# vicchu/land_trendr

Hardware: AMD Instinct MI355X
Metric: Mpixels/sec full analyze (30-yr series) (higher is better)
Workload: dtype f64

## Files before the change

### land_trendr_amd/csrc/lt_fast.h

```cpp
#pragma once
#ifndef __HIPCC_RTC__
#include <type_traits>
#endif

#include "lt_pixel.h"

#ifndef LT_WB
#define LT_WB 8
#endif
#ifndef LT_RESOLVE_PRIV_MAXY
#define LT_RESOLVE_PRIV_MAXY 48
#endif
#ifndef LT_RESOLVE_FULL
#define LT_RESOLVE_FULL 1
#endif
#ifndef LT_AB_NO_YEAR_STORES
#define LT_AB_NO_YEAR_STORES 0
#endif
#ifndef LT_AB_NO_FITS
#define LT_AB_NO_FITS 0
#endif
#ifndef LT_AB_YEAR_SINK
#define LT_AB_YEAR_SINK 0
#endif
#ifndef LT_YEAR_NT
#define LT_YEAR_NT 1
#endif
#ifndef LT_YEAR_STORE_MODE
#define LT_YEAR_STORE_MODE 0
#endif

namespace lt {
__device__ inline void year_row_store(double v, double* a) {
#if LT_YEAR_STORE_MODE == 1
  asm volatile("global_store_dwordx2 %0, %1, off sc1" ::"v"(a), "v"(v) : "memory");
#elif LT_YEAR_STORE_MODE == 2
  asm volatile("global_store_dwordx2 %0, %1, off sc0 sc1" ::"v"(a), "v"(v) : "memory");
#elif LT_YEAR_STORE_MODE == 3
  asm volatile("global_store_dwordx2 %0, %1, off sc1 nt" ::"v"(a), "v"(v) : "memory");
#else
  __builtin_nontemporal_store(v, a);
#endif
}
}
#ifndef LT_CERT_RULES
#define LT_CERT_RULES 4
#endif
#ifndef LT_PASSB_SLOTS
#define LT_PASSB_SLOTS 3
#endif

#ifdef LT_SPEC_NRULES
#define LT_NRULES LT_SPEC_NRULES
#define LT_RULE(r) lt_spec_rules[r]
#define LT_PRE_MODE LT_SPEC_PRE_MODE
#else
#define LT_NRULES P.n_rules
#define LT_RULE(r) P.rules[r]
#define LT_PRE_MODE P.pre_threshold_mode
#endif
#ifdef LT_SPEC_LINE_COST
#define LT_LINE_COST LT_SPEC_LINE_COST
#else
#define LT_LINE_COST P.line_cost
#endif

namespace lt {

__device__ inline int dmul24(int m, int sxx, int sx) {
  return (int)(__umul24((unsigned)m, (unsigned)sxx) - __umul24((unsigned)sx, (unsigned)sx));
}

__device__ inline int wave_max(int v) {
#pragma unroll
  for (int o = 32; o > 0; o >>= 1) {
    const int u = __shfl_xor(v, o);
    v = u > v ? u : v;
  }
  return __builtin_amdgcn_readfirstlane(v);
}

template <class GX, class GY>
__device__ inline int lsq_lockstep(bool act, int m, GX X, GY Y, const lsq_xf* __restrict__ xtab,
                                   bool need_solution, bool need_ssr, double& slope, double& icpt,
                                   double& ssr) {
  const int key = act ? xset_key(m, X) : 0;
  const bool miss = act && key < 0;
  lsq_xf f;
  if (act && !miss) f = xtab[key];
  if (__ballot(miss)) {
    if (miss) lsq_factor(m, X, f);
  }
  slope = 0.0;
  icpt = 0.0;
  ssr = 0.0;
  return act ? lsq_apply(f, X, Y, need_solution, need_ssr, slope, icpt, ssr) : 0;
}

template <class GX, class GY>
__device__ inline int lsq_fit_lockstep(bool act, int m, GX X, GY Y,
                                       const lsq_xf* __restrict__ xtab, double& slope,
                                       double& icpt) {
  const int key = act ? xset_key(m, X) : 0;
  const bool miss = act && key < 0;
  lsq_xf f;
  if (act && !miss) f = xtab[key];
  if (__ballot(miss)) {
    if (miss) lsq_factor(m, X, f);
  }
  slope = 0.0;
  icpt = 0.0;
  int rc = 0;
  const bool big = act && m > 4;
  if (__ballot(big)) {
    if (big) {
      double ssr;
      rc = lsq_apply(f, X, Y, true, false, slope, icpt, ssr);
    }
  }
  if (act && m <= 4) rc = lsq_apply_small(f, X, Y, slope, icpt);
  return rc;
}

template <int MAXY, class VT, bool AGLDS>
struct WaveLds {
  VT ys[MAXY][64];
  uint8_t xn[MAXY][64];
  uint8_t ag[AGLDS ? MAXY : 1][64];
  int32_t year[LT_MAX_YEARS];
};

enum { kDone = 0, kDeferExact = 1, kDeferWide = 2 };

struct NoProbe {
  static constexpr int kStopAfter = -1;
  __device__ void mark(int) const {}
};

template <int MAXY, int RMAX, bool EXACT, class VT, class Probe = NoProbe>
__device__ inline int analyze_fast(const DevScene& S_launch, const lt_params& P, const lt_tile_in& in,
                                   const lt_tile_out& out, const lsq_xf* __restrict__ xtab,
                                   uint64_t* __restrict__ yflags, uint64_t* __restrict__ tl_bits,
                                   double* __restrict__ tl_eqn, int64_t p, bool live, int lane,
                                   WaveLds<MAXY, VT, EXACT>& L,
                                   const Probe& probe = Probe()) {
#ifdef LT_SPEC_SCENE
  const DevScene& S = lt_spec_scene;
  (void)S_launch;
#else
  const DevScene& S = S_launch;
#endif
#ifdef LT_SPEC_Y
  constexpr int Y = LT_SPEC_Y;
#else
  const int Y = S.n_years;
#endif
  const int64_t is = in.stride, os = out.stride;
  const double nan = __builtin_nan("");
  int status = LT_ST_OK;
  static_assert(LT_MAX_YEARS == 64, "one year-table word per lane");
  if (lane < Y) L.year[lane] = S.year[lane];
#ifdef LT_DEBUG_LDS_POISON
  for (int k = 0; k < MAXY; k++) {
    L.ys[k][lane] = (VT)(LT_DEBUG_LDS_POISON + 37 * k);
    L.xn[k][lane] = (uint8_t)(LT_DEBUG_LDS_POISON + 11 * k);
  }
#endif
  __syncthreads();

  int T = 0, y0 = 0;
  uint64_t pres = 0;
  constexpr bool kIntSeries = std::is_same<VT, int16_t>::value;
#if defined(LT_SPEC_YEAR_OUT) && LT_SPEC_YEAR_OUT == 0
  constexpr bool kFlatPick = true;
#else
  constexpr bool kFlatPick = false;
#endif
  double Ssum = 0.0, Qsum = 0.0;
  bool f32_bad = false;
  bool intdata = true;
  bool infdata = false;
  constexpr int WB = LT_WB;
#ifdef LT_SPEC_MASKED
  constexpr bool masked = LT_SPEC_MASKED != 0;
#ifdef LT_SPEC_VBITS
  constexpr bool vbits = masked && LT_SPEC_VBITS != 0;
#else
  const bool vbits = masked && in.obs_valid_bits != nullptr && S.n_obs <= 128;
#endif
#else
  const bool masked = in.obs_valid != nullptr || in.obs_valid_bits != nullptr;
  const bool vbits = in.obs_valid_bits != nullptr && S.n_obs <= 128;
#endif
  uint32_t vw0 = 0, vw1 = 0, vw2 = 0, vw3 = 0;
  if (vbits) {
    const uint32_t* vb = in.obs_valid_bits;
    const int64_t pq = live ? p : 0;
    const int nw = (S.n_obs + 31) >> 5;
    vw0 = vb[pq];
    if (nw > 1) vw1 = vb[is + pq];
    if (nw > 2) vw2 = vb[2 * is + pq];
    if (nw > 3) vw3 = vb[3 * is + pq];
  }
  for (int yb = 0; yb < Y; yb += WB) {
    int best[WB];
#pragma unroll
    for (int u = 0; u < WB; u++) {
      const int y = yb + u;
      best[u] = -1;
      if (y >= Y) continue;
      if (!masked) {
        best[u] = live ? S.winner_all[y] : -1;
        continue;
      }
      int bd = 0x7fffffff;
      const int k1 = S.slot_begin[y + 1];
      for (int k = S.slot_begin[y]; k < k1; k++) {
// ... 423 lines not shown
            const double den = md * D;
            double r = __builtin_amdgcn_rcp(den);
            r = __builtin_fma(r, __builtin_fma(-den, r, 1.0), r);
            e = __builtin_fma(t1, D, -(N1 * N1)) * r;
            e = e < 0.0 ? 0.0 : e;
          }
          const double v = (e + c) + oi;
          if (m >= 3) w = __builtin_fma(0x1p-50, __builtin_fabs(v), kScreen * Syy);
          if (v - w <= H) cand |= 1ull << i;
          H = v + w < H ? v + w : H;
          if (prune && m >= 3 && !__ballot(col && !(dp_start_bound(e, oi, 0.0, c, SyyAll) > H)))
            break;
        }
        const int nc = col ? __builtin_popcountll(cand) : 0;
        const int ncmax = wave_max(nc);
        double best = inf;
        int bi = 0;
        for (int r = 0; r < ncmax; r++) {
          const bool act = r < nc;
          const int i = act ? __builtin_ctzll(cand) : 0;
          if (act) cand &= cand - 1;
          const double oi = OPT[i];
          const int m = j - i + 1;
          const bool ls = act && m >= 3;
          double e = 0.0;
          if (__ballot(ls)) {
            double sm, sb, ssr;
            const int rc = lsq_lockstep(
                ls, m, [&](int k) { return (int)L.xn[i + k][lane]; },
                [&](int k) { return (double)L.ys[i + k][lane]; }, xtab, false, true, sm, sb, ssr);
            if (ls) {
              if (rc < 0) status |= LT_ST_NUMERIC;
              e = ssr;
            }
          }
          const double v = (e + c) + oi;
          if (act && v < best) {
            best = v;
            bi = i;
          }
        }
        if (col) {
          ag_set(j, bi);
          OPT[j + 1] = best;
        }
      }
    } else {
      const double c = LT_LINE_COST;
      const double inf = __builtin_inf();
      double OPT[MAXY + 1];
#pragma unroll
      for (int k = 0; k <= MAXY; k++) OPT[k] = 0.0;
      double SyyAll = 0.0;
      const bool prune = c >= 0.0;
      for (int jj = 0; jj < nmax; jj++) {
        const int j = __builtin_amdgcn_readfirstlane(jj);
        const bool col = j < n;
        double Sy = 0.0, Sxy = 0.0, Syy = 0.0;
        int Sx = 0, Sxx = 0;
        double H = inf;
        uint64_t cand = 0;
        {
          const double yj = (double)L.ys[j][lane];
          SyyAll = __builtin_fma(yj, yj, SyyAll);
        }
#pragma unroll
        for (int i = MAXY - 1; i >= 0; i--) {
          if (i > j) continue;
          const int xi = L.xn[i][lane];
          const double yi = (double)L.ys[i][lane];
          Sx += xi;
          Sxx += xi * xi;
          Sy += yi;
          Sxy = __builtin_fma((double)xi, yi, Sxy);
          Syy = __builtin_fma(yi, yi, Syy);
          const int m = j - i + 1;
          double e = 0.0, w = 0.0;
          if (m >= 3) {
            const double md = (double)m;
            const double D = (double)(m * Sxx - Sx * Sx);
            const double t1 = __builtin_fma(md, Syy, -(Sy * Sy));
            const double N1 = __builtin_fma(md, Sxy, -((double)Sx * Sy));
            const double den = md * D;
            double r = __builtin_amdgcn_rcp(den);
            r = __builtin_fma(r, __builtin_fma(-den, r, 1.0), r);
            e = __builtin_fma(t1, D, -(N1 * N1)) * r;
            e = e < 0.0 ? 0.0 : e;
          }
          const double v = (e + c) + OPT[i];
          if (m >= 3) w = __builtin_fma(0x1p-50, __builtin_fabs(v), kScreen * Syy);
          if (v - w <= H) cand |= 1ull << i;
          H = v + w < H ? v + w : H;
          if (prune && m >= 3 && !__ballot(col && !(dp_start_bound(e, OPT[i], 0.0, c, SyyAll) > H)))
            break;
        }
        const int nc = col ? __builtin_popcountll(cand) : 0;
        const int ncmax = wave_max(nc);
        double best = inf;
        int bi = 0;
        for (int r = 0; r < ncmax; r++) {
          const bool act = r < nc;
          const int i = act ? __builtin_ctzll(cand) : 0;
          if (act) cand &= cand - 1;
          const int m = j - i + 1;
          const bool ls = act && m >= 3;
          double e = 0.0;
          if (__ballot(ls)) {
            double sm, sb, ssr;
            const int rc = lsq_lockstep(
                ls, m, [&](int k) { return (int)L.xn[i + k][lane]; },
                [&](int k) { return (double)L.ys[i + k][lane]; }, xtab, false, true, sm, sb, ssr);
            if (ls) {
              if (rc < 0) status |= LT_ST_NUMERIC;
              e = ssr;
            }
          }
          double o = 0.0;
#pragma unroll
          for (int k = 0; k < MAXY; k++)
            if (k == i) o = OPT[k];
          const double v = (e + c) + o;
          if (act && v < best) {
            best = v;
            bi = i;
          }
        }
        if (col) {
          ag_set(j, bi);
#pragma unroll
          for (int k = 1; k <= MAXY; k++)
            if (k == j + 1) OPT[k] = best;
        }
      }
    }
    if (n >= 1) {
      vmask = 1ull << (n - 1);
      for (int j = n - 1; j >= 0;) {
        const int a = ag_get(j);
        vmask |= 1ull << a;
        j = a - 1;
      }
    }
  } else if (nmax >= 1) {
    const double c = LT_LINE_COST;
    const double inf = __builtin_inf();
    double OPTa[MAXY + 1];
    OPTa[0] = 0.0;
    uint64_t exact = 1;
    double Emax = 0.0;
    int xA = 0, xB = 0, xC = 0, xD = 0;
    double yA = 0.0, yB = 0.0, yC = 0.0, yD = 0.0;
    double oA = 0.0, oB = 0.0, oC = 0.0, oD = 0.0;
    int gA = 0, gB = 0, gC = 0, gD = 0;
    double SyyAll = 0.0;
    const bool prune = c >= 0.0;
    const bool zok = c > 0.0;
    const bool zlane = zok && intdata;
    const uint64_t zmask = __ballot(zlane);
    uint64_t amb = 0;
    auto resolve_column = [&](const int j, const bool xr, const double H, uint64_t cs,
                              const double opt_j, const int tg_j, const double opt_jm1,
                              const int tg_jm1, int& a, double& vnew) {
      {
        const double v0 = c + opt_j;
        const double w0 = tg_j < 256 ? 0.0 : __builtin_fma(0x1p-50, __builtin_fabs(v0), Emax);
        if (!(v0 - w0 > H)) cs |= 1ull << j;
        if (j >= 1) {
          const double v1s = c + opt_jm1;
          const double w1 =
              tg_jm1 < 256 ? 0.0 : __builtin_fma(0x1p-50, __builtin_fabs(v1s), Emax);
          if (!(v1s - w1 > H)) cs |= 1ull << (j - 1);
        }
      }
      if (!xr) cs = 0;
      uint64_t need = cs & ~exact;
      {
        const int top = wave_max(need ? 63 - __builtin_clzll(need) : 0);
        for (int kk = top; kk >= 1; kk--) {
          const int k = __builtin_amdgcn_readfirstlane(kk);
          if ((need >> k) & 1) {
            const int b = L.ag[k - 1][lane];
            if (!((exact >> b) & 1)) need |= 1ull << b;
          }
        }
      }
      const int steps = wave_max(__builtin_popcountll(need) + __builtin_popcountll(cs));
      double best = inf;
      int bi = 0;
      for (int r = 0; r < steps; r++) {
        const bool link = need != 0;
        const bool act = link || cs != 0;
        int i = 0, m = 0;
        int k = 0;
        if (link) {
          k = __builtin_ctzll(need);
          need &= need - 1;
          i = L.ag[k - 1][lane];
          m = k - i;
        } else if (act) {
          i = __builtin_ctzll(cs);
          cs &= cs - 1;
          m = j - i + 1;
        }
        const bool ls = act && m >= 3;
        double e = 0.0;
        if (__ballot(ls)) {
          double sm, sb, ssr;
          const int rc = lsq_lockstep(
              ls, m, [&](int q) { return (int)L.xn[i + q][lane]; },
              [&](int q) { return (double)L.ys[i + q][lane]; }, xtab, false, true, sm, sb, ssr);
          if (ls) {
            if (rc < 0) status |= LT_ST_NUMERIC;
            e = ssr;
          }
        }
        if (act) {
          const double v = (e + c) + OPTa[i];
          if (link) {
            OPTa[k] = v;
            exact |= 1ull << k;
          } else if (v < best) {
            best = v;
            bi = i;
          }
        }
      }
      if (xr) {
        a = bi;
        vnew = best;
      }
    };
    auto column = [&](const int j, int& wx0, int& wx1, int& wx2, int& wx3, double& wy0,
                      double& wy1, double& wy2, double& wy3, double& opt_j, double& opt_jm1,
                      double& opt_jm2, double& opt_jm3, int& tg_j, int& tg_jm1, int& tg_jm2,
                      int& tg_jm3) __attribute__((always_inline)) {
      const bool col = j < n;
      const uint64_t colmask = __ballot(col);
      double Sy = 0.0, Sxy = 0.0, Syy = 0.0;
      int Sx = 0, Sxx = 0;
      double Ve = inf, Hi = inf, L1 = inf, L2 = inf, v1 = inf, gv = inf;
      double U = inf;
      int ie = 0, i1 = 0, iL = -1, n1 = -1, gi = -1, gt = 0;
      uint64_t cand = 0;
      auto track = [&](int i, double v, double hi, double lo, int nt) __attribute__((always_inline)) {
        if (hi <= Hi) {
          i1 = i;
          v1 = v;
          n1 = nt;
        }
        Hi = __builtin_fmin(hi, Hi);
        U = __builtin_fmin(U, hi);
        const bool bl = lo <= L1;
        L2 = bl ? L1 : __builtin_fmin(lo, L2);
        L1 = __builtin_fmin(lo, L1);
        iL = bl ? i : iL;
      };
      double gh = inf;
      auto zero_start = [&](int i, double v, int tg) __attribute__((always_inline)) {
        if (tg >= 0 && tg < 256) {
          if (v <= Ve) {
            Ve = v;
            ie = i;
          }
          U = __builtin_fmin(U, v);
          return;
        }
        const double w = __builtin_fma(0x1p-50, __builtin_fabs(v), Emax);
        const int ord = (!zok || tg < 0) ? 0 : gi < 0 ? 1 : tag_order(tg, gt, v, c);
        if (ord > 0) {
          gi = i;
          gt = tg;
          gv = v;
          gh = v + w;
          U = __builtin_fmin(U, gh);
        } else if (ord == 0) {
          track(i, v, v + w, v - w, tg < 0 ? -1 : tg + 1);
        }
      };
      {
        const bool has1 = j >= 1;
        const double v0 = c + opt_j, v1s = c + opt_jm1;
        const bool x0 = tg_j < 256, x1 = has1 && tg_jm1 < 256;
        const bool g0 = !x0, g1 = has1 && !x1;
        Ve = x0 ? v0 : inf;
        ie = j;
        if (x1 && v1s <= Ve) {
          Ve = v1s;
          ie = j - 1;
        }
        const int ord = (zok && g0 && g1) ? tag_order(tg_jm1, tg_j, v1s, c) : 0;
        const bool pick1 = g1 && (!g0 || ord > 0);
        gi = pick1 ? j - 1 : (g0 ? j : -1);
        gt = pick1 ? tg_jm1 : tg_j;
        gv = pick1 ? v1s : (g0 ? v0 : inf);
        gh = gv + __builtin_fma(0x1p-50, __builtin_fabs(gv), Emax);
        const bool left = g0 && g1 && ord == 0;
        if (__ballot(left)) {
          if (left) {
            const double w = __builtin_fma(0x1p-50, __builtin_fabs(v1s), Emax);
            track(j - 1, v1s, v1s + w, v1s - w, tg_jm1 + 1);
          }
        }
      }
      U = __builtin_fmin(__builtin_fmin(Hi, Ve), gh);
      wx0 = L.xn[j][lane];
      wy0 = (double)L.ys[j][lane];
      SyyAll = __builtin_fma(wy0, wy0, SyyAll);
      auto add_xy = [&](int xi, double yi) {
        Sx += xi;
        Sxx += xi * xi;
        Sy += yi;
        Sxy = __builtin_fma((double)xi, yi, Sxy);
        Syy = __builtin_fma(yi, yi, Syy);
      };
      const double slack = 4.0 * kScreen * SyyAll * (1.0 + 0x1p-49);
      auto price = [&](int i, double o, int tg, double& v, double& hi, double& lo,
                       double& bnd) __attribute__((always_inline)) {
        const int m = j - i + 1;
        const double md = (double)m;
        const double D = (double)dmul24(m, Sxx, Sx);
        const double t1 = __builtin_fma(md, Syy, -(Sy * Sy));
        const double N1 = __builtin_fma(md, Sxy, -((double)Sx * Sy));
        const double den = md * D;
        double r = __builtin_amdgcn_rcp(den);
        r = __builtin_fma(r, __builtin_fma(-den, r, 1.0), r);
        const double e = __builtin_fmax(__builtin_fma(t1, D, -(N1 * N1)) * r, 0.0);
        v = (e + c) + o;
        const double wopt = (tg >= 0 && tg < 256) ? 0.0 : Emax;
        const double ws = kScreen * Syy;
        const double w = __builtin_fma(0x1p-50, __builtin_fabs(v), ws + wopt);
        hi = v + w;
        lo = v - w;
        bnd = dp_start_bound_slack(e, o, wopt, c, slack);
        return e <= ws;
      };
      auto zero_test = [&](int m, int sx, int sxx, double sy, double sxy, double syy)
                           __attribute__((always_inline)) {
        const double md = (double)m;
        const double D = (double)dmul24(m, sxx, sx);
        const double t1 = __builtin_fma(md, syy, -(sy * sy));
        const double N1 = __builtin_fma(md, sxy, -((double)sx * sy));
        return zero_bound(wx0) * syy < 0x1p-54 * c && sse_exact_zero(t1, D, N1);
      };
      auto offer = [&](int i, double o, int tg, double v, double hi, double lo, bool zr) __attribute__((always_inline)) {
        if (zr) {
          zero_start(i, c + o, tg);
          hi = inf;
          lo = inf;
        }
        track(i, v, hi, lo, -1);
      };
      add_xy(wx0, wy0);
      if (j >= 1) add_xy(wx1, wy1);
      auto upper = [&]() __attribute__((always_inline)) { return U; };
      auto one_start = [&](int i, double o, int tg) __attribute__((always_inline)) {
        double v, hi, lo, bnd;
        const bool nz = price(i, o, tg, v, hi, lo, bnd);
        if constexpr (EXACT) {
          if (!(lo > upper())) cand |= 1ull << i;
        }
        if (__ballot(lo <= upper())) {
          if (__ballot(nz) & zmask) {
            const bool zr = zlane && nz && zero_test(j - i + 1, Sx, Sxx, Sy, Sxy, Syy);
            if (__ballot(zr)) {
              offer(i, o, tg, v, hi, lo, zr);
              return bnd;
            }
          }
          track(i, v, hi, lo, -1);
        }
        return bnd;
      };
      auto leave = [&](double bnd) __attribute__((always_inline)) {
        return prune && (__ballot(!(bnd > upper())) & colmask) == 0;
      };
      bool more = j >= 2;
      if (more) {
        add_xy(wx2, wy2);
        more = !leave(one_start(j - 2, opt_jm2, tg_jm2));
        if (j >= 3 && more) {
          add_xy(wx3, wy3);
          more = !leave(one_start(j - 3, opt_jm3, tg_jm3));
        }
        more = more && j >= 3;
      }
      if (more) {
        for (int i = __builtin_amdgcn_readfirstlane(j - 4); i >= 0;
             i = __builtin_amdgcn_readfirstlane(i - 1)) {
          add_xy(L.xn[i][lane], (double)L.ys[i][lane]);
          if (leave(one_start(i, OPTa[i], ((exact >> i) & 1) ? 0 : -1))) break;
        }
      }
      {
        const double w = __builtin_fma(0x1p-50, __builtin_fabs(gv), Emax);
        track(gi, gv, gv + w, gv - w, gt + 1);
      }
      const double H = __builtin_fmin(Hi, Ve);
      int a, tnew;
      double vnew, enew = 0.0;
      bool xres = false;
      if (L1 > H) {
        a = ie;
        vnew = Ve;
        tnew = 0;
      } else if (iL == i1 && L2 > H && Ve > H) {
        a = i1;
        vnew = v1;
        tnew = n1 >= 0 ? n1 : (j + 1) << 8;
        enew = __builtin_fma(Hi - v1, 1.0 + 0x1p-50, 0x1p-50 * __builtin_fabs(Hi));
      } else {
        if constexpr (EXACT) xres = col;
        else if (col) amb |= 1ull << j;
        a = v1 <= Ve ? i1 : ie;
        vnew = v1 <= Ve ? v1 : Ve;
        tnew = (j + 1) << 8;
        const double Lo = __builtin_fmin(L1, Ve);
        enew = (H - Lo) * (1.0 + 0x1p-40) + 0x1p-50 * __builtin_fabs(vnew);
      }
      if constexpr (EXACT) {
        if (__ballot(xres)) resolve_column(j, xres, H, cand, opt_j, tg_j, opt_jm1, tg_jm1, a, vnew);
        if (xres) {
          tnew = 0;
          enew = 0.0;
        }
      }
      if (col) {
        ag_set(j, a);
        OPTa[j + 1] = vnew;
        if (tnew < 256) exact |= 2ull << j;
        Emax = __builtin_fmax(enew, Emax);
        opt_jm3 = vnew;
        tg_jm3 = tnew;
      }
    };
    if constexpr (EXACT) {
      for (int jj = 0; jj < nmax; jj++) {
        const int j = __builtin_amdgcn_readfirstlane(jj);
        column(j, xA, xB, xC, xD, yA, yB, yC, yD, oA, oB, oC, oD, gA, gB, gC, gD);
        const int xt = xD;
        xD = xC;
        xC = xB;
        xB = xA;
        xA = xt;
        const double yt = yD;
        yD = yC;
        yC = yB;
        yB = yA;
        yA = yt;
        const double ot = oD;
        oD = oC;
        oC = oB;
        oB = oA;
        oA = ot;
        const int gt = gD;
        gD = gC;
        gC = gB;
        gB = gA;
        gA = gt;
      }
    } else
    for (int jj = 0; jj < nmax; jj += 4) {
      const int j = __builtin_amdgcn_readfirstlane(jj);
      column(j, xA, xB, xC, xD, yA, yB, yC, yD, oA, oB, oC, oD, gA, gB, gC, gD);
      if (j + 1 < nmax)
        column(j + 1, xD, xA, xB, xC, yD, yA, yB, yC, oD, oA, oB, oC, gD, gA, gB, gC);
      if (j + 2 < nmax)
        column(j + 2, xC, xD, xA, xB, yC, yD, yA, yB, oC, oD, oA, oB, gC, gD, gA, gB);
      if (j + 3 < nmax)
        column(j + 3, xB, xC, xD, xA, yB, yC, yD, yA, oB, oC, oD, oA, gB, gC, gD, gA);
    }
    if (n >= 1) {
      vmask = 1ull << (n - 1);
      for (int j = n - 1; j >= 0;) {
        const int a = ag_get(j);
        if ((amb >> j) & 1) deferred = true;
        vmask |= 1ull << a;
        j = a - 1;
      }
    }
  }
  probe.mark(2);
  if constexpr (Probe::kStopAfter == 2) return kDone;
  if (deferred) vmask = 0;

#ifdef LT_SPEC_YEAR_OUT
  constexpr bool year_out = LT_SPEC_YEAR_OUT != 0;
#else
  const bool year_out = out.val_fit || out.fit_m || out.fit_b || out.right_m || out.right_b ||
                        out.spike || out.vertex;
#endif
  RuleState1 rs[RMAX];
  double prev_fit = 0.0;
  int32_t prev_year = 0;
  auto offer_rules = [&](int q, int32_t yr, double fit_vertex) __attribute__((always_inline)) {
    if (q > 0) {
#pragma unroll
      for (int r = 0; r < RMAX; r++)
        if (r < LT_NRULES)
          rs[r].offer(LT_RULE(r), LT_PRE_MODE, prev_year, yr - prev_year, prev_fit,
                      prev_fit - fit_vertex, status);
    }
    prev_fit = fit_vertex;
    prev_year = yr;
  };
#ifdef LT_SPEC_TL_SPLIT
  constexpr bool tl_split = LT_SPEC_TL_SPLIT != 0;
#else
  const bool tl_split = tl_bits != nullptr;
#endif
  if (year_out && tl_split) {
    const bool emit = live && !deferred;
    const bool good = emit && ok;
    const uint64_t vm = good ? vmask : 0;
    const int nv = __builtin_popcountll(vm);
    const int nvmax = wave_max(nv);
    uint64_t vrem = vm, left = 0;
    double pm = 0.0, pb = 0.0;
    double* const eq = tl_eqn;
    const int64_t np = in.n_pix;
    for (int q = 0; q < nvmax; q++) {
      const bool act = q < nv;
      const int ka = act ? __builtin_ctzll(vrem) : 0;
      if (act) vrem &= vrem - 1;
      const bool has_next = act && q + 1 < nv;
      const int kb = has_next ? __builtin_ctzll(vrem) : ka;
      double cm = pm, cb = pb;
      if (__ballot(has_next)) {
        double sm = 0.0, sbv = 0.0;
        const int rc = lsq_fit_lockstep(
            has_next, has_next ? kb - ka + 1 : 2,
            [&](int k) { return (int)L.xn[(has_next ? ka : 0) + k][lane]; },
            [&](int k) { return (double)L.ys[(has_next ? ka : 0) + k][lane]; }, xtab, sm, sbv);
        if (has_next) {
          if (rc < 0) status |= LT_ST_NUMERIC;
          cm = sm;
          cb = sbv;
          typedef double d2 __attribute__((ext_vector_type(2)));
          d2 v;
          v.x = cm;
          v.y = cb;
          __builtin_nontemporal_store(v, (d2*)(eq + 2 * ((int64_t)q * np + p)));
        }
      }
      const double raw_v = act ? (double)L.ys[ka][lane] : 0.0;
      const double x = act ? (double)L.xn[ka][lane] : 0.0;
      double fit_vertex = (cm * x) + cb;
      if (q > 0 && !(pm == cm && pb == cb)) {
        const double fl = (pm * x) + pb;
        if (__builtin_fabs(fl - raw_v) <= __builtin_fabs(fit_vertex - raw_v)) {
          fit_vertex = fl;
          left |= 1ull << q;
        }
      }
      if (act) offer_rules(q, y0 + L.xn[ka][lane], fit_vertex);
      pm = cm;
      pb = cb;
    }
    if (emit) {
      __builtin_nontemporal_store(good ? pres : 0ull, tl_bits + p);
      __builtin_nontemporal_store(spike, tl_bits + np + p);
      __builtin_nontemporal_store(vm, tl_bits + 2 * np + p);
      __builtin_nontemporal_store(left, tl_bits + 3 * np + p);
    }
  } else if (year_out) {
    const bool emit = live && !deferred;
    const bool good = emit && ok;
    uint64_t vrem = vmask;
    uint64_t frem = vmask;
    double pm = 0.0, pb = 0.0;
    double cm = 0.0, cb = 0.0;
    double nm = 0.0, nb = 0.0;
    bool have_n = false;
    uint64_t spk = 0, vtx = 0;
    int t = 0, k = 0, q = 0;
    struct Row {
      double fv, fm, fb, rm, rb;
      bool pr;
      bool uni;
    };
    auto store_row = [&](int yy, const Row& r) __attribute__((always_inline)) {
      const int64_t o = LT_AB_YEAR_SINK ? p : (int64_t)yy * os + p;
      auto put = [&](double* plane, double v) __attribute__((always_inline)) {
        if (plane && !LT_AB_NO_YEAR_STORES) {
          if (LT_AB_YEAR_SINK == 2 || !LT_YEAR_NT)
            plane[o] = v;
          else
            year_row_store(v, plane + o);
        }
      };
      if (r.uni) {
        put(LT_OUTF(out, val_fit), r.fv);
        put(LT_OUTF(out, fit_m), r.fm);
        put(LT_OUTF(out, fit_b), r.fb);
        put(LT_OUTF(out, right_m), r.rm);
        put(LT_OUTF(out, right_b), r.rb);
      } else {
        put(LT_OUTF(out, val_fit), r.pr ? r.fv : nan);
        put(LT_OUTF(out, fit_m), r.pr ? r.fm : nan);
        put(LT_OUTF(out, fit_b), r.pr ? r.fb : nan);
        put(LT_OUTF(out, right_m), r.pr ? r.rm : nan);
        put(LT_OUTF(out, right_b), r.pr ? r.rb : nan);
      }
    };
    for (int y = 0; y < Y; y++) {
      const bool pr = good && ((pres >> y) & 1);
      const bool sp = pr && ((spike >> t) & 1);
      const bool isv = pr && !sp && ((vrem >> k) & 1);
      const uint64_t after = vrem & (vrem - 1);
      const bool nextfit = isv && after != 0;
      double sm = 0.0, sbv = 0.0;
      bool fitnow = false;
      if (__ballot(nextfit && !have_n) && !LT_AB_NO_FITS) {
        const uint64_t fnext = frem & (frem - 1);
        fitnow = fnext != 0 && (!have_n || nextfit);
        const int kbase = fitnow ? __builtin_ctzll(frem) : 0;
        const int kb = fitnow ? __builtin_ctzll(fnext) : 1;
        const int rc = lsq_fit_lockstep(
            fitnow, kb - kbase + 1, [&](int i) { return (int)L.xn[kbase + i][lane]; },
            [&](int i) { return (double)L.ys[kbase + i][lane]; }, xtab, sm, sbv);
        if (fitnow) {
          if (rc < 0) status |= LT_ST_NUMERIC;
          frem = fnext;
// ... 285 lines not shown
```

### land_trendr_amd/csrc/lt_pixel.h

```cpp
#pragma once
#ifndef __HIPCC_RTC__
#include <hip/hip_runtime.h>
#include <stdint.h>
#endif

#include "../../include/lt_abi.h"
#include "lt_lapack.h"

#define LT_FIELD_status (1u << 0)
#define LT_FIELD_n_years (1u << 1)
#define LT_FIELD_matched (1u << 2)
#define LT_FIELD_class_val (1u << 3)
#define LT_FIELD_onset_year (1u << 4)
#define LT_FIELD_duration (1u << 5)
#define LT_FIELD_magnitude (1u << 6)
#define LT_FIELD_initial_val (1u << 7)
#define LT_FIELD_winner (1u << 8)
#define LT_FIELD_val_raw (1u << 9)
#define LT_FIELD_val_fit (1u << 10)
#define LT_FIELD_fit_m (1u << 11)
#define LT_FIELD_fit_b (1u << 12)
#define LT_FIELD_right_m (1u << 13)
#define LT_FIELD_right_b (1u << 14)
#define LT_FIELD_spike (1u << 15)
// ... 126 lines not shown
__host__ __device__ inline double fit_width_factor(int x_max) { return x_max <= 63 ? 1.0 : 16.0; }

struct RuleState {
  bool have[LT_MAX_RULES];
  int32_t on[LT_MAX_RULES], du[LT_MAX_RULES];
  double mag[LT_MAX_RULES], init[LT_MAX_RULES];

  __host__ __device__ void reset(int nr) {
    for (int r = 0; r < nr; r++) {
      have[r] = false;
      on[r] = LT_NODATA;
      du[r] = LT_NODATA;
      mag[r] = (double)LT_NODATA;
      init[r] = (double)LT_NODATA;
    }
  }

  __host__ __device__ void offer(const lt_params& P, int32_t d_on, int32_t d_du, double d_init,
                        double d_mag, int& status) {
    for (int r = 0; r < P.n_rules; r++) {
      const lt_rule& R = P.rules[r];
      bool match = true;
      if (R.onset_op == LT_Q_EQ) match = match && ((double)d_on == R.onset_val);
      else if (R.onset_op == LT_Q_LE) match = match && !((double)d_on > R.onset_val);
      else if (R.onset_op == LT_Q_GE) match = match && !((double)d_on < R.onset_val);
      if (R.duration_op == LT_Q_GT) match = match && !((double)d_du <= R.duration_val);
      else if (R.duration_op == LT_Q_LT) match = match && !((double)d_du >= R.duration_val);
      if (R.pre_op != LT_Q_UNSET) {
        if (P.pre_threshold_mode == LT_PRE_REFERENCE) status |= LT_ST_PRE_THRESHOLD_ATTR;
        else if (R.pre_op == LT_Q_GT) match = match && !(d_init <= R.pre_val);
        else if (R.pre_op == LT_Q_LT) match = match && !(d_init >= R.pre_val);
      }
      if (!match) continue;
      bool take = !have[r];
      if (have[r]) {
        if (R.change_type == LT_CT_FD) take = d_on < on[r];
        else if (R.change_type == LT_CT_GD) take = d_mag > mag[r];
        else if (R.change_type == LT_CT_LD) take = d_du > du[r];
      }
      if (take) {
        have[r] = true;
        on[r] = d_on;
        du[r] = d_du;
        mag[r] = d_mag;
        init[r] = d_init;
      }
    }
  }

  __host__ __device__ void write(const lt_params& P, const lt_tile_out& out, int64_t p) const {
    const int64_t os = out.stride;
    for (int r = 0; r < P.n_rules; r++) {
      const int64_t q = (int64_t)r * os + p;
      if (out.matched) out.matched[q] = have[r] ? 1 : 0;
      if (out.class_val) out.class_val[q] = have[r] ? P.rules[r].class_val : LT_NODATA;
      if (out.onset_year) out.onset_year[q] = on[r];
      if (out.duration) out.duration[q] = du[r];
      if (out.magnitude) out.magnitude[q] = mag[r];
      if (out.initial_val) out.initial_val[q] = init[r];
    }
  }
};

constexpr double kScreen = 0x1p-30;

__host__ __device__ inline int lin_type_bits(int t) {
  switch (t) {
    case LT_T_I8: case LT_T_U8: return 8;
    case LT_T_I16: case LT_T_U16: return 16;
    case LT_T_I32: case LT_T_U32: return 32;
    default: return 64;
  }
}
__host__ __device__ inline bool lin_type_signed(int t) {
  return t == LT_T_I8 || t == LT_T_I16 || t == LT_T_I32 || t == LT_T_I64;
}
__host__ __device__ inline void lin_out_range(int t, int64_t& lo, int64_t& hi) {
  const int b = lin_type_bits(t);
  if (b == 64) {
    lo = (int64_t)(1ull << 63);
    hi = (int64_t)((1ull << 63) - 1);
  } else if (lin_type_signed(t)) {
    lo = -(int64_t)(1ull << (b - 1));
    hi = (int64_t)(1ull << (b - 1)) - 1;
  } else {
    lo = 0;
    hi = (int64_t)((1ull << b) - 1);
  }
}
__host__ __device__ inline double lin_store(const lt_index_lin& L, uint64_t acc) {
  const int bits = lin_type_bits(L.wrap_type);
  int64_t r = (int64_t)acc;
  if (bits < 64) {
    const int sh = 64 - bits;
    r = lin_type_signed(L.wrap_type) ? (int64_t)(acc << sh) >> sh : (int64_t)((acc << sh) >> sh);
  }
  if (L.out_type == LT_T_F64) return (double)r;
  if (L.out_type == LT_T_F32) return (double)(float)r;
  int64_t lo, hi;
  lin_out_range(L.out_type, lo, hi);
  return (double)(r < lo ? lo : r > hi ? hi : r);
}
template <class B>
__host__ __device__ inline uint64_t lin_term(int64_t coef, B b) {
  return (uint64_t)coef * (uint64_t)(int64_t)b;
}
__host__ __device__ inline double lin_value(const lt_tile_in& in, int64_t o, int64_t p) {
  const lt_index_lin& L = in.lin;
  uint64_t acc = (uint64_t)L.c0;
  for (int s = 0; s < L.n_bands && s < LT_LIN_MAX_BANDS; s++) {
    const int64_t i = o * in.band_obs_stride + s * in.band_stride + p * in.band_pix_stride;
    switch (L.band_type) {
      case LT_T_I16: acc += lin_term(L.coef[s], ((const int16_t*)in.obs_bands)[i]); break;
      case LT_T_U16: acc += lin_term(L.coef[s], ((const uint16_t*)in.obs_bands)[i]); break;
      case LT_T_U8: acc += lin_term(L.coef[s], ((const uint8_t*)in.obs_bands)[i]); break;
      default: acc += lin_term(L.coef[s], ((const int32_t*)in.obs_bands)[i]); break;
    }
  }
  return lin_store(L, acc);
}

__host__ __device__ inline bool obs_is_valid(const lt_tile_in& in, int64_t o, int64_t p) {
  if (in.obs_valid_bits) return (in.obs_valid_bits[(o >> 5) * in.stride + p] >> (o & 31)) & 1u;
  return in.obs_valid == nullptr || in.obs_valid[o * in.stride + p] != 0;
}

__host__ __device__ inline double obs_value(const lt_tile_in& in, int64_t o, int64_t p) {
  if (in.obs_bands) return lin_value(in, o, p);
  const int64_t i = o * in.stride + p;
  if (in.obs_index == nullptr) return in.obs_val[i];
  switch (in.index_type) {
    case LT_T_I16: return (double)((const int16_t*)in.obs_index)[i];
    case LT_T_U16: return (double)((const uint16_t*)in.obs_index)[i];
    case LT_T_I32: return (double)((const int32_t*)in.obs_index)[i];
    case LT_T_F32: return (double)((const float*)in.obs_index)[i];
    case LT_T_U8: return (double)((const uint8_t*)in.obs_index)[i];
    case LT_T_U32: return (double)((const uint32_t*)in.obs_index)[i];
    case LT_T_I8: return (double)((const int8_t*)in.obs_index)[i];
    case LT_T_I64: return (double)((const int64_t*)in.obs_index)[i];
    default: return ((const double*)in.obs_index)[i];
  }
}

__host__ __device__ inline double dp_start_bound_slack(double e, double opta, double eopt,
                                                       double c, double slack) {
  const double o = opta - eopt > c ? opta - eopt : c;
  return (e + o) * (1.0 - 0x1p-49) - slack;
}
__host__ __device__ inline double dp_start_bound(double e, double opta, double eopt, double c,
                                                 double SyyAll) {
  return dp_start_bound_slack(e, opta, eopt, c, 4.0 * kScreen * SyyAll * (1.0 + 0x1p-49));
}

constexpr double kZero = 0x1p-80;
constexpr double kZeroWide = 0x1p-74;
__host__ __device__ inline double zero_bound(int x_max) { return x_max <= 63 ? kZero : kZeroWide; }

__host__ __device__ inline bool sse_exact_zero(double t1, double D, double N1) {
  const double p = t1 * D, q = N1 * N1;
  return p == q && __builtin_fma(t1, D, -p) == __builtin_fma(N1, N1, -q);
}

__host__ __device__ inline int tag_order(int tn, int tg, double v, double c) {
  if ((tn >> 8) != (tg >> 8)) return 0;
  if ((tn & 255) <= (tg & 255)) return 1;
  return c > 0x1p-50 * __builtin_fabs(v) ? -1 : 0;
}

template <int MAXY>
__host__ __device__ inline void dp_screened(int n, const uint8_t* xs, const double* ys, double c,
                                   double* OPT, uint8_t* arg, int& status) {
  double va[MAXY];
  double SyyAll = 0.0;
  for (int j = 0; j < n; j++) {
    double Sy = 0.0, Sxy = 0.0, Syy = 0.0;
    int Sx = 0, Sxx = 0;
    double vmin = __builtin_inf(), wmax = 0.0, Hc = __builtin_inf();
    SyyAll += ys[j] * ys[j];
    for (int i = 0; i <= j; i++) va[i] = __builtin_inf();
    for (int i = j; i >= 0; i--) {
      const int xi = xs[i];
      const double yi = ys[i];
      Sx += xi;
      Sxx += xi * xi;
      Sy += yi;
      Sxy += (double)xi * yi;
      Syy += yi * yi;
      const int m = j - i + 1;
      double e = 0.0, w = 0.0;
      if (m >= 3) {
        const double md = (double)m;
        const double D = (double)(m * Sxx - Sx * Sx);
        const double t1 = md * Syy - Sy * Sy;
        const double N1 = md * Sxy - (double)Sx * Sy;
        e = (t1 - N1 * N1 / D) / md;
        if (e < 0.0) e = 0.0;
        w = kScreen * Syy;
      }
      const double v = (e + c) + OPT[i];
      w += 0x1p-50 * __builtin_fabs(v);
      va[i] = v;
      vmin = v < vmin ? v : vmin;
      wmax = w > wmax ? w : wmax;
      Hc = v + w < Hc ? v + w : Hc;
      if (m >= 3 && c >= 0.0 && dp_start_bound(e, OPT[i], 0.0, c, SyyAll) > Hc) break;
    }
    const double lim = vmin + 2.0 * wmax;
    double best = 0.0;
    int bi = -1;
    for (int i = 0; i <= j; i++) {
      if (!(va[i] <= lim)) continue;
      const int m = j - i + 1;
      double e = 0.0;
      if (m >= 3) {
        double sm, sb, ssr;
        int rc = lstsq_xint(
            m, [&](int k) { return (int)xs[i + k]; }, [&](int k) { return ys[i + k]; }, false,
            true, sm, sb, ssr);
        if (rc < 0) status |= LT_ST_NUMERIC;
        e = ssr;
      }
      const double v = (e + c) + OPT[i];
      if (bi < 0 || v < best) {
        best = v;
        bi = i;
      }
    }
    OPT[j + 1] = best;
    arg[j] = (uint8_t)bi;
  }
}

template <int MAXY>
__host__ __device__ inline bool dp_lazy(int n, const uint8_t* xs, const double* ys, double c,
                                        uint8_t* arg, uint64_t* amb_out = nullptr) {
  double OPTa[MAXY + 1], E[MAXY + 1];
  int TG[MAXY + 1];
  uint64_t amb = 0;
  OPTa[0] = 0.0;
  E[0] = 0.0;
  TG[0] = 0;
  bool intdata = true;
  for (int k = 0; k < n; k++)
    intdata = intdata && ys[k] == (double)(int)ys[k] && ys[k] >= -32768.0 && ys[k] <= 32767.0;
  const bool zero_ok = c > 0.0;
  double SyyAll = 0.0;
  for (int j = 0; j < n; j++) {
    SyyAll += ys[j] * ys[j];
    double Sy = 0.0, Sxy = 0.0, Syy = 0.0;
    int Sx = 0, Sxx = 0;
    const double inf = __builtin_inf();
    double Ve = inf;
    double Hi = inf, Li1 = inf, Li2 = inf, vHi = 0.0, wHi = 0.0, vbest = inf;
    int ie = -1, iHi = -1, ibest = -1, iL1 = -2, tHi = -1;
    double gv = 0.0, gw = 0.0;
    int gi = -1, gtag = 0;
    auto track = [&](int i, double v, double w, int ntag) {
      const double lo = v - w, hi = v + w;
      if (hi <= Hi) {
        Hi = hi;
        iHi = i;
        vHi = v;
        wHi = w;
        tHi = ntag;
      }
      if (lo <= Li1) {
        Li2 = Li1;
        Li1 = lo;
        iL1 = i;
      } else if (lo < Li2) {
        Li2 = lo;
      }
    };
    for (int i = j; i >= 0; i--) {
      const int xi = xs[i];
      const double yi = ys[i];
      Sx += xi;
      Sxx += xi * xi;
      Sy += yi;
      Sxy += (double)xi * yi;
      Syy += yi * yi;
      const int m = j - i + 1;
      double e = 0.0, ws = 0.0;
      bool zr = m <= 2;
      if (m >= 3) {
        const double md = (double)m;
        const double D = (double)(m * Sxx - Sx * Sx);
        const double t1 = md * Syy - Sy * Sy;
        const double N1 = md * Sxy - (double)Sx * Sy;
        e = (t1 - N1 * N1 / D) / md;
        if (e < 0.0) e = 0.0;
        ws = kScreen * Syy;
        if (zero_ok && intdata && e <= ws && zero_bound(xs[j]) * Syy < 0x1p-54 * c &&
            sse_exact_zero(t1, D, N1)) {
          zr = true;
          e = 0.0;
          ws = 0.0;
        }
      }
      const double v = (e + c) + OPTa[i];
      bool tracked = true;
      if (zr && E[i] == 0.0) {
        if (v <= Ve) {
          Ve = v;
          ie = i;
        }
      } else if (zr && zero_ok) {
        const double w = E[i] + 0x1p-50 * __builtin_fabs(v);
        const int ord = gi < 0 ? 1 : tag_order(TG[i], gtag, v, c);
        if (ord > 0) {
          gi = i;
          gtag = TG[i];
          gv = v;
          gw = w;
        } else if (ord < 0) {
          tracked = false;
        } else {
          track(i, v, w, TG[i] + 1);
        }
      } else {
        track(i, v, E[i] + ws + 0x1p-50 * __builtin_fabs(v), -1);
      }
      if (tracked && v <= vbest) {
        vbest = v;
        ibest = i;
      }
      double Hc = Hi < Ve ? Hi : Ve;
      if (gi >= 0 && gv + gw < Hc) Hc = gv + gw;
      if (m >= 3 && c >= 0.0 && dp_start_bound(e, OPTa[i], E[i], c, SyyAll) > Hc) break;
    }
    if (gi >= 0) track(gi, gv, gw, gtag + 1);
    const double H = Hi < Ve ? Hi : Ve;
    if (Li1 > H) {
      arg[j] = (uint8_t)ie;
      OPTa[j + 1] = Ve;
      E[j + 1] = 0.0;
      TG[j + 1] = 0;
    } else if (iL1 == iHi && Li2 > H && Ve > H) {
      arg[j] = (uint8_t)iHi;
      OPTa[j + 1] = vHi;
      E[j + 1] = wHi;
      TG[j + 1] = tHi >= 0 ? tHi : (j + 1) << 8;
    } else {
      TG[j + 1] = (j + 1) << 8;
      amb |= 1ull << j;
      arg[j] = (uint8_t)ibest;
      OPTa[j + 1] = vbest;
      const double L = Li1 < Ve ? Li1 : Ve;
      E[j + 1] = (H - L) * (1.0 + 0x1p-40) + 0x1p-50 * __builtin_fabs(vbest);
    }
  }
  if (amb_out) *amb_out = amb;
  for (int j = n - 1; j >= 0; j = arg[j] - 1)
    if ((amb >> j) & 1) return false;
  return true;
}

template <int MAXY, bool LAZY>
__host__ __device__ bool analyze_pixel(const DevScene& S, const lt_params& P, const lt_tile_in& in,
                                       const lt_tile_out& out, int64_t p) {
  const int Y = S.n_years;
  const int64_t is = in.stride, os = out.stride;
  int status = LT_ST_OK;

  double val[MAXY];
  uint8_t slot[MAXY];
  int T = 0;
  for (int y = 0; y < Y; y++) {
    int best = -1, bd = 0x7fffffff;
    const int k1 = S.slot_begin[y + 1];
    for (int k = S.slot_begin[y]; k < k1; k++) {
      const int o = S.order[k];
      const bool ok = obs_is_valid(in, o, p);
      if (ok && S.dist[k] < bd) {
        bd = S.dist[k];
        best = o;
      }
    }
    if (out.winner) out.winner[(int64_t)y * os + p] = (int16_t)best;
    if (best >= 0) {
      if ((S.feb29_mask >> y) & 1) status |= LT_ST_FEB29;
      val[T] = obs_value(in, (int64_t)best, p);
      slot[T] = (uint8_t)y;
      T++;
    }
  }
  if (out.n_years) out.n_years[p] = T;
  const int y0 = T > 0 ? S.year[slot[0]] : 0;

  uint64_t spike_m = 0;
  const bool ok = T >= 2;
  if (T == 0) status |= LT_ST_EMPTY;
  if (T == 1) status |= LT_ST_SINGLE_YEAR;
  const double nan = __builtin_nan("");

  {
    int t = 0;
    for (int y = 0; y < Y; y++) {
      const bool present = t < T && slot[t] == y;
      const int64_t q = (int64_t)y * os + p;
      if (!present || !ok) {
        if (out.val_raw) out.val_raw[q] = present ? val[t] : nan;
        if (out.val_fit) out.val_fit[q] = nan;
        if (out.fit_m) out.fit_m[q] = nan;
        if (out.fit_b) out.fit_b[q] = nan;
        if (out.right_m) out.right_m[q] = nan;
        if (out.right_b) out.right_b[q] = nan;
        if (out.spike) out.spike[q] = 0;
        if (out.vertex) out.vertex[q] = 0;
      }
      if (present) t++;
    }
  }

  RuleState rs;
  rs.reset(P.n_rules);

  if (ok) {
    const double avg = np_sum(T, [&](int i) { return val[i]; }) / (double)T;
    const double sd = __builtin_sqrt(np_sum(T, [&](int i) {
                                       double d = avg - val[i];
                                       return d * d;
                                     }) /
                                     (double)T);
    double last_good = val[0];
    for (int i = 1; i < T - 1; i++) {
      const double xv = val[i - 1], yv = val[i], zv = val[i + 1];
      const bool mono = (xv <= yv && yv <= zv) || (xv >= yv && yv >= zv);
      if (!mono && (__builtin_fabs(yv - xv) > sd && __builtin_fabs(yv - zv) > sd) &&
          yv != last_good) {
        spike_m |= 1ull << i;
      } else {
        last_good = yv;
      }
    }
    double ys[MAXY];
    uint8_t xs[MAXY];
    int n = 0;
    for (int i = 0; i < T; i++) {
      if ((spike_m >> i) & 1) continue;
      xs[n] = (uint8_t)(S.year[slot[i]] - y0);
      ys[n] = val[i];
      n++;
    }
#ifdef LT_HOST_DIAG
    lt_host_diag_series(p, n, xs, ys);
#endif
    uint8_t arg[MAXY];
    if constexpr (LAZY) {
      if (!dp_lazy<MAXY>(n, xs, ys, P.line_cost, arg)) return false;
    } else {
      double OPT[MAXY + 1];
      OPT[0] = 0.0;
      dp_screened<MAXY>(n, xs, ys, P.line_cost, OPT, arg, status);
    }
    uint64_t vnon = 1ull << (n - 1);
    for (int j = n - 1; j >= 0; j = arg[j] - 1) vnon |= 1ull << arg[j];

    double cm = 0.0, cb = 0.0;
    int k = 0;
    double left_fit = 0.0;
    int32_t left_year = y0;
    for (int i = 0; i < T; i++) {
      const bool sp = (spike_m >> i) & 1;
      bool is_v = false;
      const double pm = cm, pb = cb;
      if (!sp) {
        if ((vnon >> k) & 1) {
          is_v = true;
          const uint64_t later = vnon & ~((2ull << k) - 1);
          if (later) {
            const int k2 = __builtin_ctzll(later);
            double sm, sb, ssr;
            int rc = lstsq_xint(
                k2 - k + 1, [&](int q) { return (int)xs[k + q]; },
                [&](int q) { return ys[k + q]; }, true, false, sm, sb, ssr);
            if (rc < 0) status |= LT_ST_NUMERIC;
            cm = sm;
            cb = sb;
          }
        }
        k++;
      }
// ... 77 lines not shown
```

Measured before the change: 3295.

## Tighten DP early-exit bound using neighbouring start's cost

```diff
diff --git a/land_trendr_amd/csrc/lt_fast.h b/land_trendr_amd/csrc/lt_fast.h
--- a/land_trendr_amd/csrc/lt_fast.h
+++ b/land_trendr_amd/csrc/lt_fast.h
@@ -63,6 +63,12 @@
 #define LT_LINE_COST LT_SPEC_LINE_COST
 #else
 #define LT_LINE_COST P.line_cost
+#endif
+
+#if LT_DP_NEIGHBOUR && defined(LT_SPEC_NRULES)
+#define LT_DP_NB_SPEC 1
+#else
+#define LT_DP_NB_SPEC 0
 #endif
 
 namespace lt {
@@ -792,6 +798,8 @@
     double yA = 0.0, yB = 0.0, yC = 0.0, yD = 0.0;
     double oA = 0.0, oB = 0.0, oC = 0.0, oD = 0.0;
     int gA = 0, gB = 0, gC = 0, gD = 0;
+    constexpr bool NB = LT_DP_NB_SPEC != 0 && !EXACT && RMAX == 1;
+    double hA = 0.0, hB = 0.0;
     double SyyAll = 0.0;
     const bool prune = c >= 0.0;
     const bool zok = c > 0.0;
@@ -873,7 +881,7 @@
     auto column = [&](const int j, int& wx0, int& wx1, int& wx2, int& wx3, double& wy0,
                       double& wy1, double& wy2, double& wy3, double& opt_j, double& opt_jm1,
                       double& opt_jm2, double& opt_jm3, int& tg_j, int& tg_jm1, int& tg_jm2,
-                      int& tg_jm3) __attribute__((always_inline)) {
+                      int& tg_jm3, double& h1, double& h2) __attribute__((always_inline)) {
       const bool col = j < n;
       const uint64_t colmask = __ballot(col);
       double Sy = 0.0, Sxy = 0.0, Syy = 0.0;
@@ -954,8 +962,9 @@
         Syy = __builtin_fma(yi, yi, Syy);
       };
       const double slack = 4.0 * kScreen * SyyAll * (1.0 + 0x1p-49);
-      auto price = [&](int i, double o, int tg, double& v, double& hi, double& lo,
-                       double& bnd) __attribute__((always_inline)) {
+      auto price = [&](int i, double o, int tg, double eh, double ok, double wk, double& v,
+                       double& hi, double& lo, double& bnd, double& eo)
+                       __attribute__((always_inline)) {
         const int m = j - i + 1;
         const double md = (double)m;
         const double D = (double)dmul24(m, Sxx, Sx);
@@ -971,7 +980,9 @@
         const double w = __builtin_fma(0x1p-50, __builtin_fabs(v), ws + wopt);
         hi = v + w;
         lo = v - w;
-        bnd = dp_start_bound_slack(e, o, wopt, c, slack);
+        if constexpr (NB) bnd = dp_start_bound_nb_slack(e, o, wopt, eh, ok, wk, c, slack);
+        else bnd = dp_start_bound_slack(e, o, wopt, c, slack);
+        eo = e;
         return e <= ws;
       };
       auto zero_test = [&](int m, int sx, int sxx, double sy, double sxy, double syy)
@@ -993,9 +1004,10 @@
       add_xy(wx0, wy0);
       if (j >= 1) add_xy(wx1, wy1);
       auto upper = [&]() __attribute__((always_inline)) { return U; };
-      auto one_start = [&](int i, double o, int tg) __attribute__((always_inline)) {
+      auto one_start = [&](int i, double o, int tg, double eh, double ok, double wk, double& eo)
+                           __attribute__((always_inline)) {
         double v, hi, lo, bnd;
-        const bool nz = price(i, o, tg, v, hi, lo, bnd);
+        const bool nz = price(i, o, tg, eh, ok, wk, v, hi, lo, bnd, eo);
         if constexpr (EXACT) {
           if (!(lo > upper())) cand |= 1ull << i;
         }
@@ -1015,12 +1027,22 @@
         return prune && (__ballot(!(bnd > upper())) & colmask) == 0;
       };
       bool more = j >= 2;
+      double onext = 0.0, hmax = 0.0;
       if (more) {
         add_xy(wx2, wy2);
-        more = !leave(one_start(j - 2, opt_jm2, tg_jm2));
+        double e1;
+        more = !leave(one_start(j - 2, opt_jm2, tg_jm2, h1, opt_jm3, Emax, e1));
+        if constexpr (NB) {
+          hmax = __builtin_fmax(h1, h2);
+          h2 = e1;
+        }
         if (j >= 3 && more) {
+          if constexpr (NB) {
+            if (j >= 4) onext = OPTa[j - 4];
+          }
           add_xy(wx3, wy3);
-          more = !leave(one_start(j - 3, opt_jm3, tg_jm3));
+          double eo;
+          more = !leave(one_start(j - 3, opt_jm3, tg_jm3, hmax, onext, Emax, eo));
         }
         more = more && j >= 3;
       }
@@ -1028,7 +1050,13 @@
         for (int i = __builtin_amdgcn_readfirstlane(j - 4); i >= 0;
              i = __builtin_amdgcn_readfirstlane(i - 1)) {
           add_xy(L.xn[i][lane], (double)L.ys[i][lane]);
-          if (leave(one_start(i, OPTa[i], ((exact >> i) & 1) ? 0 : -1))) break;
+          double eo;
+          if constexpr (NB) {
+            const double o = onext;
+            onext = OPTa[i >= 1 ? i - 1 : 0];
+            if (leave(one_start(i, o, ((exact >> i) & 1) ? 0 : -1, hmax, onext, Emax, eo))) break;
+          } else
+          if (leave(one_start(i, OPTa[i], ((exact >> i) & 1) ? 0 : -1, 0.0, 0.0, 0.0, eo))) break;
         }
       }
       {
@@ -1076,7 +1104,7 @@
     if constexpr (EXACT) {
       for (int jj = 0; jj < nmax; jj++) {
         const int j = __builtin_amdgcn_readfirstlane(jj);
-        column(j, xA, xB, xC, xD, yA, yB, yC, yD, oA, oB, oC, oD, gA, gB, gC, gD);
+        column(j, xA, xB, xC, xD, yA, yB, yC, yD, oA, oB, oC, oD, gA, gB, gC, gD, hA, hB);
         const int xt = xD;
         xD = xC;
         xC = xB;
@@ -1101,13 +1129,13 @@
     } else
     for (int jj = 0; jj < nmax; jj += 4) {
       const int j = __builtin_amdgcn_readfirstlane(jj);
-      column(j, xA, xB, xC, xD, yA, yB, yC, yD, oA, oB, oC, oD, gA, gB, gC, gD);
+      column(j, xA, xB, xC, xD, yA, yB, yC, yD, oA, oB, oC, oD, gA, gB, gC, gD, hA, hB);
       if (j + 1 < nmax)
-        column(j + 1, xD, xA, xB, xC, yD, yA, yB, yC, oD, oA, oB, oC, gD, gA, gB, gC);
+        column(j + 1, xD, xA, xB, xC, yD, yA, yB, yC, oD, oA, oB, oC, gD, gA, gB, gC, hB, hA);
       if (j + 2 < nmax)
-        column(j + 2, xC, xD, xA, xB, yC, yD, yA, yB, oC, oD, oA, oB, gC, gD, gA, gB);
+        column(j + 2, xC, xD, xA, xB, yC, yD, yA, yB, oC, oD, oA, oB, gC, gD, gA, gB, hA, hB);
       if (j + 3 < nmax)
-        column(j + 3, xB, xC, xD, xA, yB, yC, yD, yA, oB, oC, oD, oA, gB, gC, gD, gA);
+        column(j + 3, xB, xC, xD, xA, yB, yC, yD, yA, oB, oC, oD, oA, gB, gC, gD, gA, hB, hA);
     }
     if (n >= 1) {
       vmask = 1ull << (n - 1);
diff --git a/land_trendr_amd/csrc/lt_pixel.h b/land_trendr_amd/csrc/lt_pixel.h
--- a/land_trendr_amd/csrc/lt_pixel.h
+++ b/land_trendr_amd/csrc/lt_pixel.h
@@ -302,6 +302,25 @@
   return dp_start_bound_slack(e, opta, eopt, c, 4.0 * kScreen * SyyAll * (1.0 + 0x1p-49));
 }
 
+#ifndef LT_DP_NEIGHBOUR
+#define LT_DP_NEIGHBOUR 1
+#endif
+__host__ __device__ inline double dp_start_bound_nb_slack(double e, double opta, double eopt,
+                                                          double eh, double optk, double eoptk,
+                                                          double c, double slack) {
+  const double o = opta - eopt > c ? opta - eopt : c;
+  const double ok = optk - eoptk > c ? optk - eoptk : c;
+  const double en = eh > e ? eh : e;
+  const double s0 = e + o, s1 = en + ok;
+  return (s1 > s0 ? s1 : s0) * (1.0 - 0x1p-49) - slack;
+}
+__host__ __device__ inline double dp_start_bound_nb(double e, double opta, double eopt, double eh,
+                                                    double optk, double eoptk, double c,
+                                                    double SyyAll) {
+  return dp_start_bound_nb_slack(e, opta, eopt, eh, optk, eoptk, c,
+                                 4.0 * kScreen * SyyAll * (1.0 + 0x1p-49));
+}
+
 constexpr double kZero = 0x1p-80;
 constexpr double kZeroWide = 0x1p-74;
 __host__ __device__ inline double zero_bound(int x_max) { return x_max <= 63 ? kZero : kZeroWide; }
@@ -322,7 +341,9 @@
                                    double* OPT, uint8_t* arg, int& status) {
   double va[MAXY];
   double SyyAll = 0.0;
+  double E1a = 0.0, E1b = 0.0;
   for (int j = 0; j < n; j++) {
+    double e1 = 0.0;
     double Sy = 0.0, Sxy = 0.0, Syy = 0.0;
     int Sx = 0, Sxx = 0;
     double vmin = __builtin_inf(), wmax = 0.0, Hc = __builtin_inf();
@@ -353,8 +374,18 @@
       vmin = v < vmin ? v : vmin;
       wmax = w > wmax ? w : wmax;
       Hc = v + w < Hc ? v + w : Hc;
+#if LT_DP_NEIGHBOUR
+      if (m == 3) e1 = e;
+      if (m >= 3 && c >= 0.0 && i >= 1) {
+        const double eh = m >= 4 && E1b > E1a ? E1b : E1a;
+        if (dp_start_bound_nb(e, OPT[i], 0.0, eh, OPT[i - 1], 0.0, c, SyyAll) > Hc) break;
+      }
+#else
       if (m >= 3 && c >= 0.0 && dp_start_bound(e, OPT[i], 0.0, c, SyyAll) > Hc) break;
-    }
+#endif
+    }
+    E1b = E1a;
+    E1a = e1;
     const double lim = vmin + 2.0 * wmax;
     double best = 0.0;
     int bi = -1;
@@ -395,7 +426,9 @@
     intdata = intdata && ys[k] == (double)(int)ys[k] && ys[k] >= -32768.0 && ys[k] <= 32767.0;
   const bool zero_ok = c > 0.0;
   double SyyAll = 0.0;
+  double E1a = 0.0, E1b = 0.0;
   for (int j = 0; j < n; j++) {
+    double e1 = 0.0;
     SyyAll += ys[j] * ys[j];
     double Sy = 0.0, Sxy = 0.0, Syy = 0.0;
     int Sx = 0, Sxx = 0;
@@ -477,8 +510,18 @@
       }
       double Hc = Hi < Ve ? Hi : Ve;
       if (gi >= 0 && gv + gw < Hc) Hc = gv + gw;
+#if LT_DP_NEIGHBOUR
+      if (m == 3) e1 = e;
+      if (m >= 3 && c >= 0.0 && i >= 1) {
+        const double eh = m >= 4 && E1b > E1a ? E1b : E1a;
+        if (dp_start_bound_nb(e, OPTa[i], E[i], eh, OPTa[i - 1], E[i - 1], c, SyyAll) > Hc) break;
+      }
+#else
       if (m >= 3 && c >= 0.0 && dp_start_bound(e, OPTa[i], E[i], c, SyyAll) > Hc) break;
-    }
+#endif
+    }
+    E1b = E1a;
+    E1a = e1;
     if (gi >= 0) track(gi, gv, gw, gtag + 1);
     const double H = Hi < Ve ? Hi : Ve;
     if (Li1 > H) {
```

New measurement: 3426 (median of 6 runs). 4.0% higher.
